# san-soucie/gdrf

Measured on AMD Instinct MI355X. Metric: ELBO steps/sec (+ achieved HBM GB/s on K_nm) at N=1e6,M=512,K=10,V=50, higher is better.
Workload: dtype f32; 1 GPU; configs[3] at 1 GPU(s): N=1000000 synthetic 2-D lattice (1000x1000), V=50, K=10, M=512 (32x16 grid inducing points), rbf kernel, Adam lr=1e-3, Trace_ELBO, 1 particle, jitter=1e-06, observations sharded over ranks; N=1000000, M=512, K=10, V=50, D=2, rows_per_rank=1000000, jitter_level=2, stores_T=False, mfma_mode=f16x3

## Files before the change

gdrf_amd/csrc/api.hip:

```cpp
#include "../../include/gdrf_hip.h"
#include "common.h"
#include "gemm_nt.h"
#include "gemm_tn.h"
#include "gemm_split.h"
#include "gemm_tn_topics.h"
#include "gemm_tn_topics1.h"
#include "kernels_mm.h"
#include "kernels_n.h"
#include "predict.h"
#include "predict_mc.h"
#include "predict_info.h"
#include "foldin.h"
#include "sample_counts.h"
#include "predict_cov.h"
#include "select_batch.h"
#include "rows_lds.h"
#include "rows_mfma.h"
#include "rows_vstream.h"
#include "rows_csr.h"
#include "hyper_tn.h"
#include "optim.h"

#include <algorithm>
#include <cmath>
// ... 777 lines not shown
                         snap_extra(c));
      c->prefact_valid = 1; c->prefact_jitter = jitter;
    }
    LAUNCHCHK("factorize");
    return 0;
  }

  static int knm(gdrf_ctx* c, const T* X, int64_t n, const T* Z, const T* params, T* out, int64_t ldo, hipStream_t s) {
    Z = cov_inputs<T>(c, Z, params, c->hyp, P(c->Zp), nullptr, false, s);
    StepRows r;
    if (int rc = step_inputs(c, X, n, params, s, &r)) return rc;
    X = r.X;
    ScopedTimer tm(c, 1, s);
    const int VE = Vec16<T>::N;
    const int vpr = (c->M + VE - 1) / VE, rpp = vpr <= 256 ? 256 / vpr : 1;
    int64_t blocks = (n + 4 * rpp - 1) / (4 * rpp);
    const int64_t cap = 256 * 64;
    if (blocks > cap) blocks = cap;
    if (blocks < 1) blocks = 1;
    if (ard_fwd(c))
      hipLaunchKernelGGL((knm_kernel<T, T, true, true, true>), dim3((unsigned)blocks), dim3(256), 0, s, X, n, Z, c->M, c->D, c->kind, c->hyp, out, ldo);
    else
      hipLaunchKernelGGL((knm_kernel<T, T, true, true>), dim3((unsigned)blocks), dim3(256), 0, s, X, n, Z, c->M, c->D, c->kind, c->hyp, out, ldo);
    LAUNCHCHK("knm");
    return 0;
  }

  static void split_scales(gdrf_ctx* c, int what, hipStream_t s) {
    hipLaunchKernelGGL(split_scales_kernel, dim3(1), dim3(64), 0, s, c->split == 2 ? 1 : 0, (const Hyper*)c->hyp, (const unsigned*)c->smx, c->ssc, c->K, what);
  }

  template <class SP>
  static int fwd_t_split(gdrf_ctx* c, int64_t n, int64_t rtiles, hipStream_t s) {
    if constexpr (std::is_same<T, float>::value) {
      using E = typename SP::E;
      const int Mp = c->Mp, K = c->K;
      const SplitLay SL{K};
      const int64_t nb = (int64_t)K * Mp * Mp, nw = n * Mp;
      {
        ScopedTimer tm(c, 2, s);
        hipLaunchKernelGGL(split_blocked_kernel<SP>, dim3((unsigned)((nb / 4 + 255) / 256)), dim3(256), 0, s, (const float*)c->ST, nb, Mp, Mp, (E*)c->STh, nb,
                           (const float*)c->ssc + SL.st(0));
        if (c->ssz != 8)
          hipLaunchKernelGGL(split_kernel<SP>, dim3((unsigned)((nw / 4 + 255) / 256)), dim3(256), 0, s, (const float*)c->W, nw, (E*)c->Wh,
                             (int64_t)c->ncap * Mp, (const float*)c->ssc + SL.w());
      }
      ScopedTimer tm(c, 5, s);
      const double panel = 0.625 * 2.0 * SP::NP * (double)Mp * Mp;
      const int KG = std::max(1, std::min(K, (int)(2.0 * 1024 * 1024 / panel)));
      c->forms[GDRF_FORM_FWD_T] = SP::NP == 2 ? 2 : 3; c->forms[GDRF_FORM_FWD_T_KG] = KG;
      const int64_t pairs = (rtiles + 1) / 2;
      const int rt8 = (int)((pairs + 7) / 8);
      FwdTSplitArgs<SP> a{(const E*)c->Wh, (int64_t)c->ncap * Mp, n, Mp, K, KG, rt8, (const E*)c->STh, nb, (float*)c->tt, c->ldk, (const float*)c->ssc};
      if constexpr (SP::NP == 2) {
        constexpr int lds4 = 8 * SplitCfg<SP>::IMG * 2 + 8 * GDRF_TILE * 4;
        HIPCHK(hipFuncSetAttribute((const void*)fwd_t_split_q4_kernel<SP>, hipFuncAttributeMaxDynamicSharedMemorySize, lds4));
        hipLaunchKernelGGL(fwd_t_split_q4_kernel<SP>, dim3((unsigned)(8 * K * rt8)), dim3(1024), lds4, s, a);
      } else {
        constexpr int lds2 = 6 * SplitCfg<SP>::IMG * 2;
        HIPCHK(hipFuncSetAttribute((const void*)fwd_t_split_cc_kernel<SP>, hipFuncAttributeMaxDynamicSharedMemorySize, lds2));
        hipLaunchKernelGGL(fwd_t_split_cc_kernel<SP>, dim3((unsigned)(8 * K * rt8)), dim3(512), lds2, s, a);
      }
      LAUNCHCHK("fwd_t_split");
      return 0;
    } else {
      return fail(-1, "fwd_t_split", "float arrays only");
    }
  }

  template <class SP>
  static int tn_split(gdrf_ctx* c, const float* B, const float* scale, int64_t scale_bs, int64_t n, int64_t rps, int sym, float* slab,
                      int nbatch, int ns, int ntiles, int sidx_b, int sidx_b_stride, hipStream_t s, const void* Ah = nullptr, int sidx_a = -1) {
    if constexpr (std::is_same<T, float>::value) {
      using E = typename SP::E;
      TNSplitArgs<SP> a{(const E*)(Ah ? Ah : c->Wh), (int64_t)c->ncap * c->Mp, c->Mp, B, c->Mp, scale, scale_bs, n, rps, c->Mp, sym, slab, nbatch, ns,
                        (const float*)c->ssc, sidx_a >= 0 ? sidx_a : SplitLay{c->K}.w(), sidx_b, sidx_b_stride};
      constexpr int lds = 3 * SP::NP * 32 * 128 * 2;
      HIPCHK(hipFuncSetAttribute((const void*)gemm_tn_split_kernel<SP>, hipFuncAttributeMaxDynamicSharedMemorySize, lds));
      hipLaunchKernelGGL(gemm_tn_split_kernel<SP>, dim3((unsigned)(ntiles * nbatch * ns)), dim3(256), lds, s, a);
      return 0;
    } else {
      return fail(-1, "tn_split", "float arrays only");
    }
  }

  template <class SP>
  static int wbar_split(gdrf_ctx* c, int64_t n, const T* U, int64_t rtiles, hipStream_t s) {
    if constexpr (std::is_same<T, float>::value) {
      using E = typename SP::E;
      const int Mp = c->Mp, K = c->K;
      const SplitLay SL{K};
      const int64_t nb = (int64_t)K * Mp * Mp;
      hipLaunchKernelGGL(split_blocked_kernel<SP>, dim3((unsigned)((nb / 4 + 255) / 256)), dim3(256), 0, s, (const float*)c->Bm, nb, Mp, Mp, (E*)c->Bh, nb,
                         (const float*)c->ssc + SL.b(0));
      BwdWbarSplitArgs<SP> a{(const float*)c->W, (const E*)c->Wh, (int64_t)c->ncap * Mp, n, c->M, Mp, K, (const E*)c->Bh, nb,
                             (const float*)c->vbar, (const float*)c->locbar, c->ldk, (const float*)c->asum, (const float*)U, (float*)c->Wbar,
                             (const float*)c->ssc, c->smx + SL.mx_wbar()};
      const size_t grp = SplitCfg<SP>::LDS_BYTES + (((size_t)K * GDRF_TILE * sizeof(float) + 15) & ~(size_t)15);
      const int nct_ = (Mp + GDRF_TILE - 1) / GDRF_TILE;
      if (K >= 2 && 2 * grp <= 160 * 1024) {
        const int64_t pairs = (rtiles + 1) / 2;
        const size_t tabb = ((size_t)K * GDRF_TILE * sizeof(float) + 15) & ~(size_t)15;
        const size_t lds_cc = 6 * (size_t)SplitCfg<SP>::IMG * 2 + 2 * tabb;
        if (std::is_same<SP, SplitF16>::value && K >= 2 && (Mp % 64) == 0 && 8 * (size_t)SplitCfg<SP>::IMG * 2 + 2 * tabb <= 160 * 1024) {
          if constexpr (std::is_same<SP, SplitF16>::value) {
            const size_t lds64 = 8 * (size_t)SplitCfg<SP>::IMG * 2 + 2 * tabb;
// ... 1444 lines not shown
```

gdrf_amd/csrc/gemm_split.h:

```cpp
#pragma once
#include <utility>
#include "common.h"
#include "gemm_nt.h"
#include "kernels_mm.h"

namespace gdrf {

typedef __bf16 bf16x8 __attribute__((ext_vector_type(8)));
typedef __bf16 bf16x4 __attribute__((ext_vector_type(4)));
typedef _Float16 f16x8 __attribute__((ext_vector_type(8)));
typedef _Float16 f16x4 __attribute__((ext_vector_type(4)));
typedef float f32x4 __attribute__((ext_vector_type(4)));
typedef uint32_t u32x4 __attribute__((ext_vector_type(4)));

struct SplitBf16 {
  using E = __bf16; using V8 = bf16x8; using V4 = bf16x4;
  static constexpr int NP = 3, NPROD = 6, ID = 1;
  static __device__ __forceinline__ constexpr int pa(int t) { constexpr int v[6] = {0, 1, 2, 0, 1, 0}; return v[t]; }
  static __device__ __forceinline__ constexpr int pb(int t) { constexpr int v[6] = {2, 1, 0, 1, 0, 0}; return v[t]; }
  static __device__ __forceinline__ f32x4 mma(V8 a, V8 b, f32x4 c) { return __builtin_amdgcn_mfma_f32_16x16x32_bf16(a, b, c, 0, 0, 0); }
  static __device__ __forceinline__ void split(float x, E (&p)[NP]) {
    p[0] = (__bf16)x;
    const float r1 = x - (float)p[0];
    p[1] = (__bf16)r1;
// ... 639 lines not shown
#pragma unroll
    for (int it = 0; it < 4; ++it) {
      if (kb + 4 * it < K) {
#pragma unroll
        for (int a = 0; a < 4; ++a)
#pragma unroll
          for (int b = 0; b < 4; ++b) acc[a][b] = __builtin_amdgcn_mfma_f32_16x16x4f32(av[it][a], bv[it][b], acc[a][b], 0, 0, 0);
      }
    }
  }
  __syncthreads();
  float wmax = 0.0f;
  float* tile = wbar_tile(smem, gp, L);
#pragma unroll
  for (int h = 0; h < 2; ++h) {
    wbar_tile_put(tile, acc, h, L);
#pragma unroll
    for (int i = 0; i < 8; ++i) {
      const int64_t m = m0 + L.wr * 64 + h * 32 + ((L.lane >> 4) + 4 * i);
      const int n = n0 + L.wc * 64 + (L.lane & 15) * 4;
      const f32x4 t = wbar_tile_get(tile, i, L);
      if (m < g.nrows && n < Mp) wbar_seg_store(out_base + m * Mp + n, t, as2v[h][i], wv[h][i], wmax);
    }
    asm volatile("s_waitcnt lgkmcnt(0)" ::: "memory");
  }
  if (g.wbar_max && g.nslice == 1) wave_max_publish(g.wbar_max, wmax);
}


#define GDRF_A10(p) "a" p "0", "a" p "1", "a" p "2", "a" p "3", "a" p "4", "a" p "5", "a" p "6", "a" p "7", "a" p "8", "a" p "9"
#define GDRF_A100(p) GDRF_A10(p "0"), GDRF_A10(p "1"), GDRF_A10(p "2"), GDRF_A10(p "3"), GDRF_A10(p "4"), GDRF_A10(p "5"), GDRF_A10(p "6"), \
                     GDRF_A10(p "7"), GDRF_A10(p "8"), GDRF_A10(p "9")
#define GDRF_ALL_AGPRS "a0", "a1", "a2", "a3", "a4", "a5", "a6", "a7", "a8", "a9", GDRF_A10("1"), GDRF_A10("2"), GDRF_A10("3"), GDRF_A10("4"), \
                       GDRF_A10("5"), GDRF_A10("6"), GDRF_A10("7"), GDRF_A10("8"), GDRF_A10("9"), GDRF_A100("1"), GDRF_A10("20"), GDRF_A10("21"), \
                       GDRF_A10("22"), GDRF_A10("23"), GDRF_A10("24"), "a250", "a251", "a252", "a253", "a254", "a255"
constexpr int wb1_wreg(int ks, int a, int p) { return ((ks * 8 + a) * 2 + p) * 4; }
constexpr int wb1_breg(int h, int ks, int b, int p) { return 128 + (((h * 2 + ks) * 4 + b) * 2 + p) * 4; }
template <int WA, int BA, bool ZERO> __device__ __forceinline__ void wb1_mfma(f32x4& P) {
  if constexpr (ZERO) asm volatile("v_mfma_f32_16x16x32_f16 %0, a[%c1:%c2], a[%c3:%c4], 0" : "=v"(P) : "i"(WA), "i"(WA + 3), "i"(BA), "i"(BA + 3));
  else asm volatile("v_mfma_f32_16x16x32_f16 %0, a[%c1:%c2], a[%c3:%c4], %0" : "+v"(P) : "i"(WA), "i"(WA + 3), "i"(BA), "i"(BA + 3));
}
template <int REG, int OFF> __device__ __forceinline__ void wb1_gload(const void* sbase, unsigned voff) {
  asm volatile("global_load_dwordx4 a[%c2:%c3], %0, %1 offset:%c4" : : "v"(voff), "s"(sbase), "i"(REG), "i"(REG + 3), "i"(OFF) : "memory", GDRF_ALL_AGPRS);
}
template <int REG, int OFF> __device__ __forceinline__ void wb1_ldsread(unsigned addr) {
  asm volatile("ds_read_b128 a[%c1:%c2], %0 offset:%c3" : : "v"(addr), "i"(REG), "i"(REG + 3), "i"(OFF) : "memory", GDRF_ALL_AGPRS);
}
template <int R0> __device__ __forceinline__ void wb1_update2(float& c0, float& c1, const f32x4& s, const f32x4& p) {
  asm volatile("v_fmac_f32 %0, %1, %2" : "+v"(c0) : "v"(s[R0]), "v"(p[R0]));
  asm volatile("v_fmac_f32 %0, %1, %2" : "+v"(c1) : "v"(s[R0 + 1]), "v"(p[R0 + 1]));
}
template <int N> __device__ __forceinline__ void wb1_vmcnt() { asm volatile("s_waitcnt vmcnt(%0)" : : "n"(N) : "memory"); }

template <int R>
__global__ __launch_bounds__(256, 1) void bwd_wbar_f16_w1_kernel(BwdWbarSplitArgs<SplitF16> g) {
  using SP = SplitF16;
  using CF = SplitCfg<SP>;
  using E = typename SP::E;
  static_assert(R == 2 || R == 4 || R == 8, "16 requests per block in K >= 16 / R phases");
  constexpr int PIECE = CF::PIECE;
  constexpr int WIMG = 4 * PIECE * 2;
  extern __shared__ __attribute__((aligned(16))) char smem[];
  SplitLane L;
  const int w = L.wave_u(), gp = w >> 1, wc = w & 1;
  L.wc = wc;
  const int K = g.K, Mp = g.Mp;
  const int tabf = (K + 1) * GDRF_TILE;
  float* const tab0 = reinterpret_cast<float*>(smem + 4 * WIMG);
  const int nct = (Mp + GDRF_TILE - 1) / GDRF_TILE;
  int64_t rtile; int ct;
  nt_xcd_map_paired(blockIdx.x, nct, gp, rtile, ct);
  const int64_t m0 = rtile * GDRF_TILE;
  const int n0 = ct * GDRF_TILE;
  wbar_fill_scales(g, tab0, (rtile - gp) * GDRF_TILE, L.tid);
  wbar_fill_scales(g, tab0 + tabf, (rtile - gp + 1) * GDRF_TILE, L.tid);
  tab0[(L.tid >> 7) * tabf + K * GDRF_TILE + (L.tid & 127)] = 0.0f;
  const float* const tab = tab0 + gp * tabf;

  const int nk = Mp / 64, nph = nk * K;
  const int lr = L.lr, lg = L.lg, drow = L.drow(), dq = L.dq();
  const unsigned w_lds = lds_addr(smem) + (unsigned)(gp * WIMG);
  const unsigned frag_addr = w_lds + (unsigned)(L.frag() * 2);
  const int64_t mbase = m0 < g.nrows ? m0 : 0;
  auto w_off = [&](int i) {
    const int64_t rel = (wc + 2 * i) * 16 + drow, last = g.nrows - 1 - mbase;
    unsigned v = (unsigned)(((int)(rel < last ? rel : last) * Mp + dq) * 2);
    asm volatile("" : "+v"(v));
    return v;
  };
  const unsigned vw0 = w_off(0), vw1 = w_off(1), vw2 = w_off(2), vw3 = w_off(3);
  const E* const w_row = g.Wh + mbase * Mp;
  auto dma_w = [&](int q, int buf, int rep_c, auto jc) {
    constexpr int j = decltype(jc)::value;
    const int r = rep_c * R + j, ks = r >> 3, p = (r >> 2) & 1;
    const unsigned va = (j & 1) ? vw1 : vw0, vb = (j & 1) ? vw3 : vw2;
    const unsigned vo = R >= 4 ? ((j & 2) ? vb : va) : ((rep_c & 1) ? vb : va);
    const int rbk = wc + 2 * (r & 3);
    const E* src = w_row + (p ? g.w_stride : 0) + q * 64 + ks * 32;
    const unsigned dst = w_lds + (unsigned)(buf * 2 * WIMG + (ks * 2 + p) * PIECE * 2 + rbk * 1024);
    asm volatile("s_mov_b32 m0, %2\n\ts_nop 4\n\tglobal_load_lds_dwordx4 %0, %1" : : "v"(vo), "s"(src), "s"(dst) : "memory");
  };
  const int col0 = (n0 + wc * 64 < Mp) ? n0 + wc * 64 : 0;
  const unsigned voff_b = (unsigned)((lr * 32 + 8 * lg) * 2);
  const int64_t b_ks = (int64_t)Mp * 32, b_rep = (int64_t)(Mp >> 5) * b_ks;
  const E* sb[2][2];
  auto b_bases = [&](const E* b0) {
    sb[0][0] = b0; sb[1][0] = b0 + b_ks; sb[0][1] = b0 + g.piece_stride; sb[1][1] = b0 + b_ks + g.piece_stride;
#pragma unroll
    for (int i = 0; i < 4; ++i) asm volatile("" : "+s"(sb[i >> 1][i & 1]));
  };
  const E* b_blk = g.Bh + (int64_t)col0 * 32;
  const E* b_cur = b_blk;

  float acc[8][4][4];
  f32x4 P[8], s8[8];
#pragma unroll
  for (int a = 0; a < 8; ++a) {
    P[a] = f32x4{0, 0, 0, 0}; s8[a] = f32x4{0, 0, 0, 0};
#pragma unroll
    for (int b = 0; b < 4; ++b)
#pragma unroll
      for (int r = 0; r < 4; ++r) acc[a][b][r] = 0.0f;
  }
  for (int rp = 0; rp < 16 / R; ++rp) static_for<R>([&](auto jc) { dma_w(0, 0, rp, jc); });
  b_bases(b_cur);
  static_for<16>([&](auto jc) {
    constexpr int j = decltype(jc)::value, bb = j >> 2, ks = (j >> 1) & 1, p = j & 1;
    wb1_gload<wb1_breg(0, ks, bb, p), bb * 1024>(sb[ks][p], voff_b);
  });
  wb1_vmcnt<0>();
  __syncthreads();

  constexpr int N1 = R / 2, N2 = R / 2;
  int c = 0, q = 0, rep = 0;
  for (int it = 0; it < (nph + 1) / 2; ++it) {
    static_for<2>([&](auto hc) {
      constexpr int h = decltype(hc)::value;
      const bool live = c < nph;
      const int qq = q < nk ? q : nk - 1;
      if (live && rep == 0) {
        if (c > 0) { wb1_vmcnt<0>(); gdrf_raw_barrier(); }
        const unsigned fa = frag_addr + (unsigned)((qq & 1) * 2 * WIMG);
        static_for<32>([&](auto fc) {
          constexpr int f = decltype(fc)::value, ks = f >> 4, p = (f >> 3) & 1, a = f & 7;
          wb1_ldsread<wb1_wreg(ks, a, p), ((ks * 2 + p) * PIECE + a * 16 * 32) * 2>(fa);
        });
        asm volatile("s_waitcnt lgkmcnt(0)" ::: "memory");
      }
      const unsigned saddr = lds_addr(tab + (live ? rep : K) * GDRF_TILE + lg * 4);
      const E* const b_next = c + 1 >= nph ? b_cur : (rep + 1 == K ? b_blk + 2 * b_ks : b_cur + b_rep);
      b_bases(b_next);
      const int qn = qq + 1 < nk ? qq + 1 : nk - 1, bufn = (qq + 1) & 1;
      const int rep_c = (live && rep < 16 / R) ? rep : 16 / R - 1;
      static_for<4>([&](auto bc) {
// ... 95 lines not shown
#pragma unroll
  for (int hr = 0; hr < 2; ++hr)
#pragma unroll
    for (int a = 0; a < 4; ++a)
      asm volatile("s_nop 15" : "+v"(accv[hr][a][0]), "+v"(accv[hr][a][1]), "+v"(accv[hr][a][2]), "+v"(accv[hr][a][3]));
  __syncthreads();
  float wmax = 0.0f;
  L.wave = w;
  float* tile = wbar_tile(smem, 0, L);
#pragma unroll
  for (int hr = 0; hr < 2; ++hr) {
    L.wr = hr;
#pragma unroll
    for (int h = 0; h < 2; ++h) {
      wbar_tile_put(tile, accv[hr], h, L);
      if (hr == 0 && h == 1) { load_w(1); L.wr = 0; }
#pragma unroll
      for (int i = 0; i < 8; ++i) {
        const int64_t m = m0 + wbar_seg_row(L, h, i);
        const int n = n0 + wbar_seg_col(L);
        const f32x4 t = wbar_tile_get(tile, i, L);
        if (m < g.nrows && n < Mp) wbar_seg_store(g.Wbar + m * Mp + n, t, as2v[hr][h][i], wv[hr][h][i], wmax);
      }
      asm volatile("s_waitcnt lgkmcnt(0)" ::: "memory");
    }
  }
  if (g.wbar_max) wave_max_publish(g.wbar_max, wmax);
}

__global__ __launch_bounds__(256) void wbar_slab_sum_kernel(const float* __restrict__ slab, int64_t slab_stride, int nslice, int64_t n4 ,
                                                           float* __restrict__ Wbar, unsigned* __restrict__ wbar_max) {
  const int64_t i = (int64_t)blockIdx.x * blockDim.x + threadIdx.x;
  float wmax = 0.0f;
  if (i < n4) {
    f32x4 acc = *reinterpret_cast<const f32x4*>(slab + 4 * i);
    for (int sl = 1; sl < nslice; ++sl) {
      const f32x4 t = *reinterpret_cast<const f32x4*>(slab + (int64_t)sl * slab_stride + 4 * i);
#pragma unroll
      for (int e = 0; e < 4; ++e) acc[e] += t[e];
    }
    *reinterpret_cast<f32x4*>(Wbar + 4 * i) = acc;
#pragma unroll
    for (int e = 0; e < 4; ++e) wmax = fmaxf(wmax, fabsf(acc[e]));
  }
  if (wbar_max) wave_max_publish(wbar_max, wmax);
}

template <class SP> struct FwdTSplitArgs {
  const typename SP::E* Wh; int64_t w_stride; int64_t nrows; int Mp, K;
  int KG; int rt8;
  const typename SP::E* STh; int64_t piece_stride;
  float* tt; int64_t ldt;
  const float* sc;
};

template <class SP> __device__ __forceinline__ void fwd_t_map_block(const FwdTSplitArgs<SP>& g, int64_t& rt0, int& bz) {
  const unsigned xcd = blockIdx.x & 7u, idx = blockIdx.x >> 3;
  const unsigned per_group = (unsigned)g.KG * (unsigned)g.rt8;
  const int grp = (int)(idx / per_group);
  const unsigned rem = idx - (unsigned)grp * per_group;
  const int kg = min(g.KG, g.K - grp * g.KG);
  rt0 = 2 * ((int64_t)(rem / (unsigned)kg) * 8 + xcd);
  bz = grp * g.KG + (int)(rem % (unsigned)kg);
}
__device__ __forceinline__ bool fwd_t_col_ok(int ct, int b, int Mp, const SplitLane& L) { return ct * GDRF_TILE + L.wc * 64 + b * 16 + L.lr < Mp; }
__device__ __forceinline__ float fwd_t_sq(float x, bool cok) { return cok ? x * x : 0.0f; }
template <class SP> __device__ __forceinline__ void fwd_t_store_tt(const FwdTSplitArgs<SP>& g, int bz, int64_t m0, int tid, float v) {
  const int64_t m = m0 + tid;
  const SplitLay SL{g.K};
  const float un = g.sc[SL.w() + 1] * g.sc[SL.st(bz) + 1];
  if (m < g.nrows) g.tt[(int64_t)bz * g.ldt + m] = v * (un * un);
}


template <class SP>
__global__ __launch_bounds__(512, 2) void fwd_t_split_cc_kernel(FwdTSplitArgs<SP> g) {
  using CF = SplitCfg<SP>;
  using E = typename SP::E;
  using V8 = typename SP::V8;
  constexpr int NP = SP::NP;
  extern __shared__ __attribute__((aligned(16))) char smem[];
  constexpr int IMG = CF::IMG;
  const int gp = __builtin_amdgcn_readfirstlane((int)(threadIdx.x >> 8));
  E* As = reinterpret_cast<E*>(smem) + gp * 2 * IMG;
  E* Bs = reinterpret_cast<E*>(smem) + 4 * IMG;
  const int Mp = g.Mp;
  const int nct = (Mp + GDRF_TILE - 1) / GDRF_TILE;
  int64_t rt0; int bz;
  fwd_t_map_block(g, rt0, bz);
  const int64_t m0 = (rt0 + gp) * GDRF_TILE;
  const SplitLane L;
  const int tid = L.tid, wr = L.wr, wc = L.wc, lr = L.lr, lg = L.lg;

  const int drow = L.drow(), dq = L.dq(), wave_u = L.wave_u();
  const unsigned a_lds = lds_addr(As), b_lds = lds_addr(Bs);
  auto dma1 = [&](int ct, int kA, int buf, int slot) {
    if (slot < 2 * NP) {
      const int i = slot / NP, p = slot - i * NP;
      const int rbk = wave_u + 4 * i;
      int64_t row = m0 + rbk * 16 + drow;
      row = row < g.nrows ? row : 0;
      glds16_asm(g.Wh + p * g.w_stride + row * Mp + kA + dq, a_lds + (unsigned)(((buf * NP + p) * CF::PIECE + rbk * 512) * 2));
    } else {
      const int p = slot - 2 * NP;
      const int rbk = wave_u + 4 * gp, row = rbk * 16 + drow;
      const int col = (ct * GDRF_TILE + row < Mp) ? ct * GDRF_TILE + row : 0;
      glds16_asm(g.STh + p * g.piece_stride + (((int64_t)bz * (Mp >> 5) + (kA >> 5)) * Mp + col) * 32 + dq,
                 b_lds + (unsigned)(((buf * NP + p) * CF::PIECE + rbk * 512) * 2));
    }
  };
  auto dma = [&](int ct, int kA, int buf) {
#pragma unroll
    for (int sl = 0; sl < 3 * NP; ++sl) dma1(ct, kA, buf, sl);
  };
  float rs[4][4];
#pragma unroll
  for (int a = 0; a < 4; ++a)
#pragma unroll
    for (int r = 0; r < 4; ++r) rs[a][r] = 0;
// ... 148 lines not shown
    }
#pragma unroll 1
    for (; kA < Mp; kA += CF::BK) {
      int cp1, kA1;
      next_chunk(cp, kA, cp1, kA1);
      const E* Ab = Asm + (gr * 2 + buf) * IMG;
      const E* Bb = Bsm + (gc * 2 + buf) * IMG;
#pragma unroll
      for (int sl = 0; sl < 2 * NP; ++sl) dma1(cp1, kA1, buf ^ 1, sl);
      V8 fb[NP][4];
#pragma unroll
      for (int p = 0; p < NP; ++p)
#pragma unroll
        for (int b = 0; b < 4; ++b) fb[p][b] = split_frag<SP>(Bb, p, wc * 64 + b * 16, frag);
#pragma unroll
      for (int a = 0; a < 4; ++a) {
        __builtin_amdgcn_sched_barrier(0);
        V8 fa[NP];
        split_frags<SP>(fa, Ab, wr * 64 + a * 16, frag);
#pragma unroll
        for (int t = 0; t < SP::NPROD; ++t)
#pragma unroll
          for (int b = 0; b < 4; ++b) acc[a][b] = SP::mma(fa[SP::pa(t)], fb[SP::pb(t)][b], acc[a][b]);
      }
      split_phase_end();
      buf ^= 1;
    }
    if (ct < nct) {
#pragma unroll
      for (int b = 0; b < 4; ++b) {
        const bool cok = fwd_t_col_ok(ct, b, Mp, L);
#pragma unroll
        for (int a = 0; a < 4; ++a) {
#pragma unroll
          for (int r = 0; r < 4; ++r) acc[a][b][r] = fwd_t_sq(acc[a][b][r], cok);
        }
      }
#pragma unroll
      for (int a = 0; a < 4; ++a) {
#pragma unroll
        for (int r = 0; r < 4; ++r) {
          const float v = group16_sum((acc[a][0][r] + acc[a][1][r]) + (acc[a][2][r] + acc[a][3][r]));
          if (lr == 0) rsum[wr * 64 + a * 16 + lg * 4 + r] += v;
        }
#pragma unroll
        for (int b = 0; b < 4; ++b) acc[a][b] = f32x4{0, 0, 0, 0};
      }
    }
  }
  __syncthreads();
  if (gc == 0 && tid < GDRF_TILE) {
    const float* q = reinterpret_cast<const float*>(smem + (size_t)8 * IMG * 2) + (gr * 2) * 2 * GDRF_TILE + tid;
    fwd_t_store_tt(g, bz, m0, tid, (q[0] + q[GDRF_TILE]) + (q[2 * GDRF_TILE] + q[3 * GDRF_TILE]));
  }
}

template <class SP> struct TNSplitArgs {
  const typename SP::E* Ah; int64_t a_stride; int64_t lda;
  const float* B; int64_t ldb;
  const float* scale; int64_t scale_bs;
  int64_t nrows, rows_per_split;
  int ncols, sym;
  float* slab;
  int nbatch, nsplit;
  const float* sc; int sidx_a;
  int sidx_b, sidx_b_stride;
};

__device__ __forceinline__ int tnb_code(int k) { return (((k >> 3) & 1) << 2) | (k & 3); }
__device__ __forceinline__ int tnb_seg(int k, int c4) { return k * 32 + (c4 ^ (tnb_code(k) << 2)); }

__device__ __forceinline__ bf16x4 tr_read(const __bf16* p) {
  return __builtin_amdgcn_ds_read_tr16_b64_v4bf16((__attribute__((address_space(3))) bf16x4*)p);
}
__device__ __forceinline__ f16x4 tr_read(const _Float16* p) {
  typedef __fp16 h4 __attribute__((__vector_size__(4 * sizeof(__fp16))));
  return __builtin_bit_cast(f16x4, __builtin_amdgcn_ds_read_tr16_b64_v4f16((__attribute__((address_space(3))) h4*)p));
}

template <class SP>
__global__ __launch_bounds__(256, 2) __attribute__((amdgpu_num_vgpr(96))) void gemm_tn_split_kernel(TNSplitArgs<SP> g) {
  using E = typename SP::E;
  using V8 = typename SP::V8;
  using V4 = typename SP::V4;
  constexpr int NP = SP::NP;
  constexpr int PIECE = 32 * 128;
  extern __shared__ __attribute__((aligned(16))) char smem[];
  E* As = reinterpret_cast<E*>(smem);
  E* Bs = As + 2 * NP * PIECE;
  const int tid = threadIdx.x, lane = tid & 63, wave = tid >> 6;
  const int wr = wave >> 1, wc = wave & 1, lr = lane & 15, lg = lane >> 4;
  const int nt = (g.ncols + GDRF_TILE - 1) / GDRF_TILE;
  const int ntiles = g.sym ? nt * (nt + 1) / 2 : nt * nt;
  int tile, b, sp;
  {
    const unsigned bid = blockIdx.x;
    if ((g.nsplit & 7) == 0) {
      const unsigned xcd = bid & 7u, idx = bid >> 3, per = (unsigned)(ntiles * g.nbatch);
      const unsigned sl = idx / per, r = idx - sl * per;
      sp = (int)(sl * 8u + xcd); b = (int)(r / (unsigned)ntiles); tile = (int)(r % (unsigned)ntiles);
    } else {
      tile = (int)(bid % (unsigned)ntiles);
      const unsigned r = bid / (unsigned)ntiles;
      b = (int)(r % (unsigned)g.nbatch); sp = (int)(r / (unsigned)g.nbatch);
    }
  }
// ... 131 lines not shown
```

gdrf_amd/engine.py:

```python
from __future__ import annotations

import contextlib
import ctypes as C
import math
from typing import Dict, Optional

import torch

from . import _lib
from .data import check_counts, is_sparse_counts

KERNEL_IDS = {"rbf": 0, "matern52": 1, "matern32": 2, "exponential": 3, "rationalquadratic": 4, "periodic": 5, "product": 6}
PRODUCT_KINDS = {"rbf": 0, "periodic": 5}
OPT_MODES = {"adam": 0, "adamw": 1, "clippedadam": 2}
OPT_RULES = {"adam": 0, "adamw": 1, "clippedadam": 2, "adamax": 3, "rmsprop": 4, "adagrad": 5, "adadelta": 6, "asgd": 7, "rprop": 8,
             "adagradrmsprop": 9}
OPT_CLIP_NORM, OPT_CLIP_VALUE, OPT_MOMENTUM, OPT_CENTERED = 1, 2, 4, 8

_WS_IDS = dict(W=0, Wbar=1, q=2, loc=3, tt=4, vbar=5, locbar=6, asum=7, Kuu=8, L=9, Linv=10, S=11, B=12, phi=13,
               mu=14, LinvT=15, ST=16, Knm=17, g_locbar=18)


def _stream_ptr(device) -> int:
    return torch.cuda.current_stream(device).cuda_stream
# ... 363 lines not shown
            y = self.Z.clamp(min=fi.tiny, max=1.0 - fi.eps)
            self.view("inducing_unc").copy_(y.log() - (-y).log1p())

    def refresh_inducing(self):
        if self.learn_inducing:
            torch.sigmoid(self.view("inducing_unc"), out=self.Z)

    def set_dirichlet(self, alpha: torch.Tensor):
        a = alpha.detach().to("cpu", torch.float64).contiguous()
        assert a.shape == (self.K, self.V)
        arr = (C.c_double * (self.K * self.V))(*a.flatten().tolist())
        _lib.check(self.lib.gdrf_set_dirichlet(self.ctx, arr), "gdrf_set_dirichlet")

    def workspace(self, name: str, n_rows: Optional[int] = None) -> torch.Tensor:
        ptr, cnt = C.c_void_p(), C.c_int64()
        _lib.check(self.lib.gdrf_ws_ptr(self.ctx, _WS_IDS[name], C.byref(ptr), C.byref(cnt)), "gdrf_ws_ptr")
        esz = self.lib.gdrf_ws_elem_size(self.ctx, _WS_IDS[name])
        flat = torch.empty(cnt.value, dtype=torch.float32 if esz == 4 else torch.float64, device=self.device)
        _lib.check(self.lib.gdrf_ws_copy(self.ctx, _WS_IDS[name], flat.data_ptr(), cnt.value, _stream_ptr(self.device)),
                   "gdrf_ws_copy")
        torch.cuda.synchronize(self.device)
        Mp = (self.M + 31) // 32 * 32
        ldk = (self.n_cap + 3) // 4 * 4
        n = self.n_cap if n_rows is None else n_rows
        if name in ("W", "Wbar", "Knm"):
            return flat.view(self.n_cap, Mp)[:n, :self.M].clone()
        if name in ("q", "asum"):
            return flat[:n].clone()
        if name in ("loc", "tt", "vbar", "locbar", "mu"):
            return flat.view(self.K, ldk)[:, :n].clone()
        if name in ("Kuu", "L", "Linv", "LinvT"):
            return flat.view(Mp, Mp)[:self.M, :self.M].clone()
        if name in ("S", "B", "ST"):
            return flat.view(self.K, Mp, Mp)[:, :self.M, :self.M].clone()
        if name == "phi":
            return flat.view(self.K, self.V).clone()
        raise KeyError(name)

    TIMING_SLOTS = ("probe", "k_nm", "transforms", "fwd_w", "loc", "fwd_t", "elbo_rows", "bwd_wbar", "bwd_knm",
                    "tn_sym", "tn_gt", "slab_reduce", "ubar", "step_finish", "adam", "factorize")

    def set_timing(self, enable: bool):
        _lib.check(self.lib.gdrf_set_timing(self.ctx, 1 if enable else 0), "gdrf_set_timing")

    def get_timing(self) -> Dict[str, Dict[str, float]]:
        n = len(self.TIMING_SLOTS)
        ms, cnt = (C.c_double * n)(), (C.c_int64 * n)()
        _lib.check(self.lib.gdrf_get_timing(self.ctx, ms, cnt, n), "gdrf_get_timing")
        return {name: dict(ms=ms[i], count=cnt[i]) for i, name in enumerate(self.TIMING_SLOTS)}

    FORM_SLOTS = ("wbar", "wbar_nslice", "a_k", "a_k_kgroups", "fwd_t", "fwd_t_kg", "loc", "ubar_q4", "rows", "rows_kt", "rows_vt", "gt",
                  "hyper", "predict", "predict_nb")
    FORM_NAMES = dict(wbar=("gemm_nt", "gemm_nt_t", "split<1>", "split<2>", "split_cc", "k64", "w1"), a_k=("gemm_tn", "tn_split", "tn_topics", "w2"),
                      fwd_t=("gemm_nt", "q4", "cc"), loc=("rows", "gemm_nt", "gemm_nt_wide"), rows=("mfma", "thread", "streamed"),
                      gt=("gemm_tn", "tn_split"), hyper=("f64", "tn"), predict=("mfma", "rows_lds", "rows_mem", "rows_bigk", "streamed"))

    def last_forms(self) -> Dict[str, object]:
        n = len(self.FORM_SLOTS)
        arr = (C.c_int * n)()
        _lib.check(self.lib.gdrf_last_forms(self.ctx, arr, n), "gdrf_last_forms")
        out = {}
        for slot, v in zip(self.FORM_SLOTS, arr):
            if v:
                out[slot] = self.FORM_NAMES[slot][v - 1] if slot in self.FORM_NAMES else v
        return out

    def _chk_rows(self, xs: torch.Tensor, ws: Optional[torch.Tensor] = None):
        if xs.device != self.device or xs.dtype != self.dtype or not xs.is_contiguous() or xs.dim() != 2 or xs.shape[1] != self.D:
            raise ValueError(f"xs must be a contiguous ({'n'},{self.D}) {self.dtype} tensor on {self.device}")
        if ws is not None and is_sparse_counts(ws):
            check_counts(ws, xs.shape[0], self.V, self.device)
        elif ws is not None:
            if ws.device != self.device or ws.dtype != torch.int32 or not ws.is_contiguous() or ws.shape != (xs.shape[0], self.V):
                raise ValueError(f"ws must be a contiguous (n,{self.V}) int32 tensor on {self.device}")

    def _counts_ptr(self, ws: Optional[torch.Tensor]):
        if ws is None or not is_sparse_counts(ws):
            if self._csr_bound:
                _lib.check(self.lib.gdrf_bind_counts_csr(self.ctx, None, None, None, 0, 0, None, None), "gdrf_bind_counts_csr")
                self._csr_bound = False
            return None if ws is None else ws.data_ptr()
        c = self._csr_cache
        if c is None or c[0] is not ws or c[1] != ws._version:
            crow = ws.crow_indices().to(torch.int64).contiguous()
            col = ws.col_indices().to(torch.int32).contiguous()
            val = ws.values().contiguous()
            order = torch.sort(col, stable=True)
            cperm = order.indices.to(torch.int64).contiguous()
            ccol = torch.searchsorted(order.values, torch.arange(self.V + 1, dtype=torch.int32, device=self.device)).to(torch.int64).contiguous()
            c = self._csr_cache = (ws, ws._version, (crow, col, val, ccol, cperm))
            self._csr_bound = False
        if not self._csr_bound:
            crow, col, val, ccol, cperm = c[2]
            _lib.check(self.lib.gdrf_bind_counts_csr(self.ctx, crow.data_ptr(), col.data_ptr(), val.data_ptr(), ws.shape[0], col.numel(),
                                                     ccol.data_ptr(), cperm.data_ptr()), "gdrf_bind_counts_csr")
            self._csr_bound = True
        return None

    def knm(self, xs: torch.Tensor) -> torch.Tensor:
        self._chk_rows(xs)
        out = torch.empty(xs.shape[0], self.M, dtype=self.dtype, device=self.device)
        self.knm_into(xs, out)
        return out

    def knm_into(self, xs: torch.Tensor, out: torch.Tensor):
        _lib.check(self.lib.gdrf_knm(self.ctx, xs.data_ptr(), xs.shape[0], self.Z.data_ptr(), self.params.data_ptr(),
                                     out.data_ptr(), out.shape[1], _stream_ptr(self.device)), "gdrf_knm")
# ... 518 lines not shown
```

Baseline: 24.83 steps/s.

## Add register-resident f16 w1 kernel for forward-T split GEMM

Adds a new fwd_t_f16_w1 kernel for the f16 split path. It holds the ST operand fragments in a VGPR ring and keeps the W image in LDS through direct global_load_lds DMA, double-buffered. Topics are processed in quads, with pairs for the remainder, and row sums are reduced with DPP. The W-image request logic is pulled out of the bwd_wbar w1 kernel into a shared W1Image helper. The aim is better W reuse across topics and better MFMA/load overlap, at the cost of a lot of fragile hand-scheduled inline asm and register clobbers.

```diff
diff --git a/gdrf_amd/csrc/api.hip b/gdrf_amd/csrc/api.hip
--- a/gdrf_amd/csrc/api.hip
+++ b/gdrf_amd/csrc/api.hip
@@ -853,6 +853,28 @@
       const int64_t pairs = (rtiles + 1) / 2;
       const int rt8 = (int)((pairs + 7) / 8);
       FwdTSplitArgs<SP> a{(const E*)c->Wh, (int64_t)c->ncap * Mp, n, Mp, K, KG, rt8, (const E*)c->STh, nb, (float*)c->tt, c->ldk, (const float*)c->ssc};
+      if constexpr (std::is_same<SP, SplitF16>::value) {
+        const int nct_ = (Mp + GDRF_TILE - 1) / GDRF_TILE;
+        if ((Mp % 64) == 0 && K >= 2 && K <= 16 && pairs * nct_ > 32) {
+          const int KQ = K / 4 * 4;
+          if (KQ) {
+            a.k_lo = 0; a.k_n = KQ; a.KG = 1; a.rt8 = (int)((rtiles + 7) / 8);
+            constexpr int lds_q = 2 * W1_WIMG + 16 * GDRF_TILE * 4;
+            HIPCHK(hipFuncSetAttribute((const void*)fwd_t_f16_w1_kernel<true>, hipFuncAttributeMaxDynamicSharedMemorySize, lds_q));
+            hipLaunchKernelGGL(fwd_t_f16_w1_kernel<true>, dim3((unsigned)(8 * (KQ / 4) * a.rt8)), dim3(256), lds_q, s, a);
+          }
+          const int KP = (K - KQ + 1) / 2, KGP = std::min(KP, FWD_T_W1_KGP);
+          if (KP) {
+            a.k_lo = KQ; a.k_n = K - KQ; a.KG = KGP; a.rt8 = rt8;
+            constexpr int lds_p = 4 * W1_WIMG + 16 * GDRF_TILE * 4;
+            HIPCHK(hipFuncSetAttribute((const void*)fwd_t_f16_w1_kernel<false>, hipFuncAttributeMaxDynamicSharedMemorySize, lds_p));
+            hipLaunchKernelGGL(fwd_t_f16_w1_kernel<false>, dim3((unsigned)(8 * KP * rt8)), dim3(256), lds_p, s, a);
+          }
+          c->forms[GDRF_FORM_FWD_T] = 4; c->forms[GDRF_FORM_FWD_T_KG] = KQ ? 4 : 2 * KGP;
+          LAUNCHCHK("fwd_t_split");
+          return 0;
+        }
+      }
       if constexpr (SP::NP == 2) {
         constexpr int lds4 = 8 * SplitCfg<SP>::IMG * 2 + 8 * GDRF_TILE * 4;
         HIPCHK(hipFuncSetAttribute((const void*)fwd_t_split_q4_kernel<SP>, hipFuncAttributeMaxDynamicSharedMemorySize, lds4));
diff --git a/gdrf_amd/csrc/gemm_split.h b/gdrf_amd/csrc/gemm_split.h
--- a/gdrf_amd/csrc/gemm_split.h
+++ b/gdrf_amd/csrc/gemm_split.h
@@ -715,6 +715,41 @@
 }
 template <int N> __device__ __forceinline__ void wb1_vmcnt() { asm volatile("s_waitcnt vmcnt(%0)" : : "n"(N) : "memory"); }
 
+constexpr int W1_WIMG = 4 * SplitCfg<SplitF16>::PIECE * 2;
+template <int NW> struct W1Image {
+  static_assert(NW == 2 || NW == 4, "row blocks per wave: 4 or 2");
+  static constexpr int PER = 8 / NW;
+  const _Float16* w_row; int64_t w_stride;
+  unsigned w_lds, buf_stride;
+  int wsub;
+  unsigned vw0, vw1, vw2, vw3;
+  __device__ __forceinline__ W1Image(const _Float16* Wh, int64_t w_stride_, int64_t nrows, int Mp, int64_t m0, unsigned w_lds_, unsigned buf_stride_, int wsub_,
+                                     const SplitLane& L)
+      : w_stride(w_stride_), w_lds(w_lds_), buf_stride(buf_stride_), wsub(wsub_) {
+    const int drow = L.drow(), dq = L.dq();
+    const int64_t mbase = m0 < nrows ? m0 : 0;
+    auto w_off = [&](int i) {
+      const int64_t rel = (wsub + NW * i) * 16 + drow, last = nrows - 1 - mbase;
+      unsigned v = (unsigned)(((int)(rel < last ? rel : last) * Mp + dq) * 2);
+      asm volatile("" : "+v"(v));
+      return v;
+    };
+    vw0 = w_off(0); vw1 = w_off(1);
+    if constexpr (NW == 2) { vw2 = w_off(2); vw3 = w_off(3); } else { vw2 = 0; vw3 = 0; }
+    w_row = Wh + mbase * Mp;
+  }
+  template <int R, int J> __device__ __forceinline__ void request(int q, int buf, int rep_c) const {
+    static_assert(NW == 2 || R % 2 == 0, "the row block must follow from J");
+    const int r = rep_c * R + J, ks = r / (2 * PER), p = (r / PER) & 1;
+    const unsigned va = (J & 1) ? vw1 : vw0, vb = (J & 1) ? vw3 : vw2;
+    const unsigned vo = NW == 4 ? va : (R >= 4 ? ((J & 2) ? vb : va) : ((rep_c & 1) ? vb : va));
+    const int rbk = wsub + NW * (r & (PER - 1));
+    const _Float16* src = w_row + (p ? w_stride : 0) + q * 64 + ks * 32;
+    const unsigned dst = w_lds + (unsigned)buf * buf_stride + (unsigned)((ks * 2 + p) * SplitCfg<SplitF16>::PIECE * 2 + rbk * 1024);
+    asm volatile("s_mov_b32 m0, %2\n\ts_nop 4\n\tglobal_load_lds_dwordx4 %0, %1" : : "v"(vo), "s"(src), "s"(dst) : "memory");
+  }
+};
+
 template <int R>
 __global__ __launch_bounds__(256, 1) void bwd_wbar_f16_w1_kernel(BwdWbarSplitArgs<SplitF16> g) {
   using SP = SplitF16;
@@ -741,28 +776,11 @@
   const float* const tab = tab0 + gp * tabf;
 
   const int nk = Mp / 64, nph = nk * K;
-  const int lr = L.lr, lg = L.lg, drow = L.drow(), dq = L.dq();
+  const int lr = L.lr, lg = L.lg;
   const unsigned w_lds = lds_addr(smem) + (unsigned)(gp * WIMG);
   const unsigned frag_addr = w_lds + (unsigned)(L.frag() * 2);
-  const int64_t mbase = m0 < g.nrows ? m0 : 0;
-  auto w_off = [&](int i) {
-    const int64_t rel = (wc + 2 * i) * 16 + drow, last = g.nrows - 1 - mbase;
-    unsigned v = (unsigned)(((int)(rel < last ? rel : last) * Mp + dq) * 2);
-    asm volatile("" : "+v"(v));
-    return v;
-  };
-  const unsigned vw0 = w_off(0), vw1 = w_off(1), vw2 = w_off(2), vw3 = w_off(3);
-  const E* const w_row = g.Wh + mbase * Mp;
-  auto dma_w = [&](int q, int buf, int rep_c, auto jc) {
-    constexpr int j = decltype(jc)::value;
-    const int r = rep_c * R + j, ks = r >> 3, p = (r >> 2) & 1;
-    const unsigned va = (j & 1) ? vw1 : vw0, vb = (j & 1) ? vw3 : vw2;
-    const unsigned vo = R >= 4 ? ((j & 2) ? vb : va) : ((rep_c & 1) ? vb : va);
-    const int rbk = wc + 2 * (r & 3);
-    const E* src = w_row + (p ? g.w_stride : 0) + q * 64 + ks * 32;
-    const unsigned dst = w_lds + (unsigned)(buf * 2 * WIMG + (ks * 2 + p) * PIECE * 2 + rbk * 1024);
-    asm volatile("s_mov_b32 m0, %2\n\ts_nop 4\n\tglobal_load_lds_dwordx4 %0, %1" : : "v"(vo), "s"(src), "s"(dst) : "memory");
-  };
+  const W1Image<2> WI(g.Wh, g.w_stride, g.nrows, Mp, m0, w_lds, 2 * WIMG, wc, L);
+  auto dma_w = [&](int q, int buf, int rep_c, auto jc) { WI.template request<R, decltype(jc)::value>(q, buf, rep_c); };
   const int col0 = (n0 + wc * 64 < Mp) ? n0 + wc * 64 : 0;
   const unsigned voff_b = (unsigned)((lr * 32 + 8 * lg) * 2);
   const int64_t b_ks = (int64_t)Mp * 32, b_rep = (int64_t)(Mp >> 5) * b_ks;
@@ -964,6 +982,7 @@
   const typename SP::E* STh; int64_t piece_stride;
   float* tt; int64_t ldt;
   const float* sc;
+  int k_lo = 0, k_n = 0;
 };
 
 template <class SP> __device__ __forceinline__ void fwd_t_map_block(const FwdTSplitArgs<SP>& g, int64_t& rt0, int& bz) {
@@ -977,6 +996,16 @@
 }
 __device__ __forceinline__ bool fwd_t_col_ok(int ct, int b, int Mp, const SplitLane& L) { return ct * GDRF_TILE + L.wc * 64 + b * 16 + L.lr < Mp; }
 __device__ __forceinline__ float fwd_t_sq(float x, bool cok) { return cok ? x * x : 0.0f; }
+__device__ __forceinline__ float row16_sum_lane0(float v) {
+  auto rot = [](float x, auto nc) {
+    return __builtin_bit_cast(float, __builtin_amdgcn_update_dpp(0, __builtin_bit_cast(int, x), 0x120 + decltype(nc)::value, 0xf, 0xf, false));
+  };
+  v += rot(v, std::integral_constant<int, 8>{});
+  v += rot(v, std::integral_constant<int, 4>{});
+  v += rot(v, std::integral_constant<int, 2>{});
+  v += rot(v, std::integral_constant<int, 1>{});
+  return v;
+}
 template <class SP> __device__ __forceinline__ void fwd_t_store_tt(const FwdTSplitArgs<SP>& g, int bz, int64_t m0, int tid, float v) {
   const int64_t m = m0 + tid;
   const SplitLay SL{g.K};
@@ -1231,6 +1260,197 @@
   if (gc == 0 && tid < GDRF_TILE) {
     const float* q = reinterpret_cast<const float*>(smem + (size_t)8 * IMG * 2) + (gr * 2) * 2 * GDRF_TILE + tid;
     fwd_t_store_tt(g, bz, m0, tid, (q[0] + q[GDRF_TILE]) + (q[2 * GDRF_TILE] + q[3 * GDRF_TILE]));
+  }
+}
+
+constexpr int FWD_T_W1_KGP = 2;
+constexpr int ft1_acc(int tp, int a, int b) { return ((tp * 8 + a) * 4 + b) * 4; }
+#define GDRF_V10(p) "v" p "0", "v" p "1", "v" p "2", "v" p "3", "v" p "4", "v" p "5", "v" p "6", "v" p "7", "v" p "8", "v" p "9"
+#define GDRF_RING_VGPRS "v192", "v193", "v194", "v195", "v196", "v197", "v198", "v199", GDRF_V10("20"), GDRF_V10("21"), GDRF_V10("22"), \
+                        GDRF_V10("23"), GDRF_V10("24"), "v250", "v251", "v252", "v253", "v254", "v255"
+#define GDRF_W1_VGPRS "v64", "v65", "v66", "v67", "v68", "v69", GDRF_V10("7"), GDRF_V10("8"), GDRF_V10("9"), GDRF_V10("10"), GDRF_V10("11"), \
+                      GDRF_V10("12"), GDRF_V10("13"), GDRF_V10("14"), GDRF_V10("15"), GDRF_V10("16"), GDRF_V10("17"), GDRF_V10("18"), "v190", "v191", \
+                      GDRF_RING_VGPRS
+constexpr int ft1_wreg(int ks, int a, int p) { return 64 + ((ks * 8 + a) * 2 + p) * 4; }
+constexpr int ft1_rreg(int b, int ks, int p) { return 192 + ((b * 2 + ks) * 2 + p) * 4; }
+template <int D, int WA, int RB, bool ZERO, bool CLOB> __device__ __forceinline__ void ft1_mfma() {
+  if constexpr (ZERO && CLOB)
+    asm volatile("v_mfma_f32_16x16x32_f16 a[%c0:%c1], v[%c2:%c3], v[%c4:%c5], 0" : : "i"(D), "i"(D + 3), "i"(WA), "i"(WA + 3), "i"(RB), "i"(RB + 3) : GDRF_ALL_AGPRS, GDRF_W1_VGPRS);
+  else if constexpr (ZERO)
+    asm volatile("v_mfma_f32_16x16x32_f16 a[%c0:%c1], v[%c2:%c3], v[%c4:%c5], 0" : : "i"(D), "i"(D + 3), "i"(WA), "i"(WA + 3), "i"(RB), "i"(RB + 3));
+  else if constexpr (CLOB)
+    asm volatile("v_mfma_f32_16x16x32_f16 a[%c0:%c1], v[%c2:%c3], v[%c4:%c5], a[%c0:%c1]" : : "i"(D), "i"(D + 3), "i"(WA), "i"(WA + 3), "i"(RB), "i"(RB + 3) : GDRF_ALL_AGPRS, GDRF_W1_VGPRS);
+  else
+    asm volatile("v_mfma_f32_16x16x32_f16 a[%c0:%c1], v[%c2:%c3], v[%c4:%c5], a[%c0:%c1]" : : "i"(D), "i"(D + 3), "i"(WA), "i"(WA + 3), "i"(RB), "i"(RB + 3));
+}
+template <int REG, int OFF> __device__ __forceinline__ void ft1_gload(const void* sbase, unsigned voff) {
+  asm volatile("global_load_dwordx4 v[%c2:%c3], %0, %1 offset:%c4" : : "v"(voff), "s"(sbase), "i"(REG), "i"(REG + 3), "i"(OFF) : "memory", GDRF_W1_VGPRS);
+}
+template <int REG, int OFF> __device__ __forceinline__ void ft1_ldsread(unsigned addr) {
+  asm volatile("ds_read_b128 v[%c1:%c2], %0 offset:%c3" : : "v"(addr), "i"(REG), "i"(REG + 3), "i"(OFF) : "memory", GDRF_W1_VGPRS);
+}
+template <int REG> __device__ __forceinline__ float ft1_accread() {
+  float x;
+  asm volatile("v_accvgpr_read_b32 %0, a[%c1]" : "=v"(x) : "i"(REG) : GDRF_ALL_AGPRS, GDRF_RING_VGPRS);
+  return x;
+}
+
+template <bool QUAD>
+__global__ __launch_bounds__(256, 1) void fwd_t_f16_w1_kernel(FwdTSplitArgs<SplitF16> g) {
+  using SP = SplitF16;
+  using CF = SplitCfg<SP>;
+  using E = typename SP::E;
+  constexpr int PIECE = CF::PIECE, WIMG = W1_WIMG;
+  extern __shared__ __attribute__((aligned(16))) char smem[];
+  constexpr int NT = QUAD ? 1 : 2, G = QUAD ? 4 : 2;
+  constexpr int RS_TP = QUAD ? 4 : 8;
+  SplitLane L;
+  const int w = L.wave_u(), gp = w >> 1, wc = w & 1;
+  L.wc = wc;
+  const int Mp = g.Mp;
+  const int nk = Mp / 64, nct = (Mp + GDRF_TILE - 1) / GDRF_TILE;
+  FwdTSplitArgs<SP> gm = g;
+  gm.K = (g.k_n + G - 1) / G;
+  int64_t rt0; int bp;
+  fwd_t_map_block(gm, rt0, bp);
+  if constexpr (QUAD) rt0 >>= 1;
+  const int k_end = g.k_lo + g.k_n, kw = g.k_lo + G * bp + (QUAD ? 2 * gp : 0);
+  const int k0 = min(kw, k_end - 1), k1 = min(kw + 1, k_end - 1);
+  const int64_t m0 = (rt0 + (QUAD ? 0 : gp)) * GDRF_TILE;
+  const int lr = L.lr, lg = L.lg;
+  const unsigned w_lds = lds_addr(smem) + (unsigned)(QUAD ? 0 : gp * WIMG);
+  const unsigned frag_addr = w_lds + (unsigned)(L.frag() * 2);
+  const W1Image<QUAD ? 4 : 2> WI(g.Wh, g.w_stride, g.nrows, Mp, m0, w_lds, NT * WIMG, QUAD ? w : wc, L);
+  constexpr int NREQ = 32 / (QUAD ? 4 : 2), RQ = NREQ / 2, NG = RQ / 2;
+  float* const rs_base = reinterpret_cast<float*>(smem + 2 * NT * WIMG);
+  float* const rs_wave = rs_base + ((QUAD ? gp * 8 : gp * 4) + wc) * GDRF_TILE;
+#pragma unroll
+  for (int i = 0; i < 4; ++i) {
+    rs_wave[((i >> 1) * RS_TP + 2 * (i & 1)) * GDRF_TILE + L.lane] = 0.0f;
+    rs_wave[((i >> 1) * RS_TP + 2 * (i & 1)) * GDRF_TILE + 64 + L.lane] = 0.0f;
+  }
+
+  const unsigned voff_b = (unsigned)((lr * 32 + 8 * lg) * 2);
+  const int64_t b_ks = (int64_t)Mp * 32, b_top = (int64_t)(Mp >> 5) * b_ks;
+  const int64_t dtop = (int64_t)(k1 - k0) * b_top;
+  const E* const st0 = g.STh + (int64_t)k0 * b_top;
+  const int64_t p_stride = g.piece_stride;
+  auto phase_base = [&](int ct, int q) {
+    const int col = ct * GDRF_TILE + wc * 64;
+    return st0 + (int64_t)(2 * q) * b_ks + (int64_t)(col < Mp ? col : ct * GDRF_TILE) * 32;
+  };
+  const E* sb[2][2];
+  auto b_bases = [&](const E* b0) {
+    sb[0][0] = b0; sb[1][0] = b0 + b_ks; sb[0][1] = b0 + p_stride; sb[1][1] = b0 + b_ks + p_stride;
+#pragma unroll
+    for (int i = 0; i < 4; ++i) asm volatile("" : "+s"(sb[i >> 1][i & 1]));
+  };
+
+
+  static_for<NREQ>([&](auto jc) { WI.template request<RQ, decltype(jc)::value % RQ>(0, 0, decltype(jc)::value / RQ); });
+  const E* b_cur = phase_base(0, wc < nk ? wc : 0);
+  b_bases(b_cur);
+  static_for<16>([&](auto jc) {
+    constexpr int j = decltype(jc)::value, bb = j >> 2, ks = (j >> 1) & 1, p = j & 1;
+    ft1_gload<ft1_rreg(bb, ks, p), bb * 1024>(sb[ks][p], voff_b);
+  });
+  wb1_vmcnt<0>();
+  __syncthreads();
+
+  auto block_body = [&](auto firstc, int qn, int bufn, const E* next_blk, unsigned fa) {
+    constexpr bool FIRST = decltype(firstc)::value;
+    auto wread = [&](auto fc) {
+      constexpr int f = decltype(fc)::value, ks = (f >> 3) & 1, p = (f >> 2) & 1, a = (f >> 4) * 4 + (f & 3);
+      ft1_ldsread<ft1_wreg(ks, a, p), ((ks * 2 + p) * PIECE + a * 16 * 32) * 2>(fa);
+    };
+    static_for<8>(wread);
+    static_for<2>([&](auto tc) {
+      constexpr int tp = decltype(tc)::value;
+      const E* const b_next = tp == 0 ? b_cur + dtop : next_blk;
+      b_bases(b_next);
+      static_for<4>([&](auto bc) {
+        constexpr int b = decltype(bc)::value;
+        wb1_vmcnt<(b & 1) ? 12 + 2 * NG : 12 + NG>();
+        static_for<48>([&](auto mc) {
+          constexpr int m = decltype(mc)::value, half = m / 24, mm = m % 24, ks = mm / 12, t = (mm >> 2) % 3, a = half * 4 + (mm & 3);
+          if constexpr (tp == 0 && b == 0) {
+            if constexpr (m == 0 || m == 4 || m == 36) asm volatile("s_waitcnt lgkmcnt(4)" ::: "memory");
+            if constexpr (m == 12 || m == 16 || m == 28) asm volatile("s_waitcnt lgkmcnt(8)" ::: "memory");
+            if constexpr (m == 24) asm volatile("s_waitcnt lgkmcnt(12)" ::: "memory");
+            if constexpr (m == 40) asm volatile("s_waitcnt lgkmcnt(0)" ::: "memory");
+          }
+          ft1_mfma<ft1_acc(tp, a, b), ft1_wreg(ks, a, SP::pa(t)), ft1_rreg(b, ks, SP::pb(t)), FIRST && mm < 4, m == 0>();
+          if constexpr (tp == 0 && b == 0 && m < 24) wread(std::integral_constant<int, 8 + m>{});
+          if constexpr ((b == 0 || b == 2) && m < 6 * NG && m % 6 == 2) WI.template request<RQ, (b == 0 ? 0 : NG) + (m - 2) / 6>(qn, bufn, tp);
+          if constexpr (m == 27) ft1_gload<ft1_rreg(b, 0, 1), b * 1024>(sb[0][1], voff_b);
+          if constexpr (m == 35) ft1_gload<ft1_rreg(b, 0, 0), b * 1024>(sb[0][0], voff_b);
+          if constexpr (m == 39) ft1_gload<ft1_rreg(b, 1, 1), b * 1024>(sb[1][1], voff_b);
+          if constexpr (m == 47) ft1_gload<ft1_rreg(b, 1, 0), b * 1024>(sb[1][0], voff_b);
+        });
+      });
+      b_cur = b_next;
+    });
+  };
+
+  int ct = 0, q = 0, s = 0;
+  bool sat = false;
+#pragma unroll 1
+  for (;;) {
+    int ctn = ct, qn = q + 1;
+    bool more = true;
+    if (qn >= nk) {
+      ctn = ct + 1; qn = 2 * ctn;
+      if (ctn >= nct) { more = false; ctn = ct; qn = q; }
+    }
+    const int bufn = (s + 1) & 1;
+    if (s > 0) {
+      if (sat) wb1_vmcnt<0>(); else wb1_vmcnt<8>();
+      gdrf_raw_barrier();
+    }
+    if (q >= 2 * ct + wc) {
+      const E* next_blk = b_cur + dtop;
+      if (q + 1 < nk) next_blk = phase_base(ct, q + 1);
+      else if (ct + 1 < nct && 2 * (ct + 1) + wc < nk) next_blk = phase_base(ct + 1, 2 * (ct + 1) + wc);
+      const unsigned fa = frag_addr + (unsigned)((s & 1) * NT * WIMG);
+      if (q == 2 * ct + wc) block_body(std::true_type{}, qn, bufn, next_blk, fa);
+      else block_body(std::false_type{}, qn, bufn, next_blk, fa);
+      sat = false;
+    } else {
+      static_for<NREQ>([&](auto jc) { WI.template request<RQ, decltype(jc)::value % RQ>(qn, bufn, decltype(jc)::value / RQ); });
+      sat = true;
+    }
+    if (q == nk - 1) {
+      asm volatile("s_nop 15\n\ts_nop 15" ::: "memory");
+      float* const slot = rs_wave + 2 * (ct & 1) * GDRF_TILE + lg * 4;
+      bool cok[4];
+#pragma unroll
+      for (int b = 0; b < 4; ++b) cok[b] = fwd_t_col_ok(ct, b, Mp, L);
+      static_for<16>([&](auto ic) {
+        constexpr int tp = decltype(ic)::value >> 3, a = decltype(ic)::value & 7;
+        f32x4 v;
+        static_for<4>([&](auto rc) {
+          constexpr int r = decltype(rc)::value;
+          const float x0 = fwd_t_sq(ft1_accread<ft1_acc(tp, a, 0) + r>(), cok[0]), x1 = fwd_t_sq(ft1_accread<ft1_acc(tp, a, 1) + r>(), cok[1]);
+          const float x2 = fwd_t_sq(ft1_accread<ft1_acc(tp, a, 2) + r>(), cok[2]), x3 = fwd_t_sq(ft1_accread<ft1_acc(tp, a, 3) + r>(), cok[3]);
+          v[r] = row16_sum_lane0((x0 + x1) + (x2 + x3));
+        });
+        if (lr == 0) {
+          f32x4* const p = reinterpret_cast<f32x4*>(slot + tp * RS_TP * GDRF_TILE + a * 16);
+          *p = *p + v;
+        }
+      });
+    }
+    if (!more) break;
+    ct = ctn; q = qn; ++s;
+  }
+  wb1_vmcnt<0>();
+  __syncthreads();
+  for (int e = L.tid; e < 4 * GDRF_TILE; e += 256) {
+    const int sl = e >> 7, row = e & 127;
+    const int kt = g.k_lo + G * bp + (QUAD ? sl : sl >> 1);
+    const float* qd = rs_base + sl * 4 * GDRF_TILE + row;
+    if (kt < k_end)
+      fwd_t_store_tt(g, kt, (rt0 + (QUAD ? 0 : sl & 1)) * GDRF_TILE, row, (qd[0] + qd[GDRF_TILE]) + (qd[2 * GDRF_TILE] + qd[3 * GDRF_TILE]));
   }
 }
 
diff --git a/gdrf_amd/engine.py b/gdrf_amd/engine.py
--- a/gdrf_amd/engine.py
+++ b/gdrf_amd/engine.py
@@ -439,7 +439,7 @@
     FORM_SLOTS = ("wbar", "wbar_nslice", "a_k", "a_k_kgroups", "fwd_t", "fwd_t_kg", "loc", "ubar_q4", "rows", "rows_kt", "rows_vt", "gt",
                   "hyper", "predict", "predict_nb")
     FORM_NAMES = dict(wbar=("gemm_nt", "gemm_nt_t", "split<1>", "split<2>", "split_cc", "k64", "w1"), a_k=("gemm_tn", "tn_split", "tn_topics", "w2"),
-                      fwd_t=("gemm_nt", "q4", "cc"), loc=("rows", "gemm_nt", "gemm_nt_wide"), rows=("mfma", "thread", "streamed"),
+                      fwd_t=("gemm_nt", "q4", "cc", "w1"), loc=("rows", "gemm_nt", "gemm_nt_wide"), rows=("mfma", "thread", "streamed"),
                       gt=("gemm_tn", "tn_split"), hyper=("f64", "tn"), predict=("mfma", "rows_lds", "rows_mem", "rows_bigk", "streamed"))
 
     def last_forms(self) -> Dict[str, object]:
```

After: 25.23 steps/s, median of 6. +1.6%, better.
